# lionelblonde/sac-td3-cudagraphs-pytorch

Hardware: AMD Instinct MI355X
Metric: gradient-steps/sec (SAC, batch=256) at 1 GPU + 8-seed node; replay HBM GB/s (higher is better)
Workload: dtype f32; 1 GPU; SAC Hopper-v4 batch=256 2x256 MLP+LN, 100000 rows in a 1000000-row HBM ring, 1 critic update+Polyak per iteration, 2 actor+alpha updates every 3rd, hipGraph per 3 iterations; parallelism=1 independent seeds, one per GPU, no collective

## Files before the change

### sac-td3-cudagraphs-pytorch_amd/csrc/engine.hip

```cpp
#include <hip/hip_runtime.h>

#include <algorithm>
#include <cmath>
#include <cstdio>
#include <cstdlib>
#include <cstring>
#include <string>
#include <chrono>
#include <vector>

#include "../../include/sactd3.h"
#include "kernels.h"

static thread_local std::string g_create_error;

static inline int round_up(int x, int m) { return (x + m - 1) / m * m; }
static inline unsigned magic_div(unsigned d, unsigned long long n_max) {
  return (d > 1 && n_max * d < (1ull << 32)) ? (unsigned)(((1ull << 32) + d - 1) / d) : 0u;
}

static NetLayout make_layout(int K, int nh) {
  NetLayout L{};
  L.K = K; L.ld1 = round_up(K, 4); L.nh = nh;
  int off = 0;
// ... 52 lines not shown

  int o = 0, a = 0, B = 0, ldc = 0, ldo = 0, a4 = 0, nh = 0, ldu = 0, rec_f = 0, rec4 = 0, cx = 0, cn = 0;
  int nq_actor = 2;
  int nblk = 0, nblk4 = 0;
  AlphaArgs pending_alpha{}; bool alpha_pending = false;
  bool alpha_tick_owed = false;
  int maxn = 0;
  int num_cus = 256;
  int stage_rows = 0;
  NetLayout La{}, Lc{};

  DevCtl* ctl = nullptr;
  float *min_ac = nullptr, *max_ac = nullptr, *scale = nullptr, *bias = nullptr;
  float *Pa = nullptr, *Ta = nullptr, *Ga = nullptr, *Ma = nullptr, *Va = nullptr;
  float *Ta2 = nullptr, *Ta3 = nullptr;
  float *Pc = nullptr, *Tc = nullptr, *Gc = nullptr, *Mc = nullptr, *Vc = nullptr;
  float *la = nullptr, *gscale = nullptr;
  float* ring = nullptr; float* stage_dev = nullptr;
  float *X = nullptr, *Xn = nullptr, *Xp = nullptr, *rew = nullptr, *done = nullptr;
  int* idx = nullptr;
  float *logp_n = nullptr, *logp_pi = nullptr, *logp_al = nullptr, *act_scratch = nullptr;
  float* eps[SACTD3_NUM_SITES] = {};
  float *a_z1 = nullptr, *a_xh1 = nullptr, *a_h1 = nullptr, *a_rs1 = nullptr, *a_z2 = nullptr, *a_xh2 = nullptr, *a_h2 = nullptr, *a_rs2 = nullptr, *a_tg = nullptr;
  float *a_du = nullptr, *a_dz2 = nullptr, *a_dh1 = nullptr, *a_dz1 = nullptr;
  float *qa_ps = nullptr, *qa_S = nullptr;
  float *a_ps = nullptr, *c_ps = nullptr;
  float* a_z2n = nullptr;
  float* ah_z1[4] = {}; float* ah_z2[4] = {};
  struct BatchSlot { float *X, *Xn, *rew, *done, *logp_n, *eps_c; int* idx; } bs[4] = {};
  int cur_slot = 0;
  int chain_ready = -1;
  float *c_z1 = nullptr, *c_xh1 = nullptr, *c_h1 = nullptr, *c_rs1 = nullptr, *c_z2 = nullptr, *c_dz2 = nullptr, *c_dh1 = nullptr, *c_dz1 = nullptr;
  float *t_z1 = nullptr, *t_z2 = nullptr, *q = nullptr, *qt = nullptr, *y = nullptr, *q_pi = nullptr, *dA = nullptr;
  float* s_h1 = nullptr;
  float* Gp = nullptr; int gp_slabs = 0;
  float *part = nullptr, *part_s = nullptr, *part_sa = nullptr;
  float *p_x = nullptr, *p_z1 = nullptr, *p_z2 = nullptr, *p_act = nullptr;
  float *h_obs = nullptr, *h_act = nullptr;
  int* h_done = nullptr; int predict_calls = 0;
  float* h_stage[NSTAGE] = {}; int stage_next = 0, stage_used = 0;
  float* h_batch = nullptr;

  int64_t rb_len = 0, rb_cursor = 0, qnet_updates = 0;
  hipGraphExec_t graphs[G_COUNT] = {}; int graph_nodes[G_COUNT] = {};
  std::vector<hipGraphExec_t> predict_graphs;
  int tune_ks = 0, tune_nt = 0, tune_tn_kt = 0, tune_pad64 = 0, tune_tn64_min = 0, tune_rows4 = 0, tune_nn16 = 0, tune_xr = -1;
  int node_seq = 0, node_only = -1;
  const char* node_role = "";
  std::vector<NodeInfo>* node_log = nullptr;

  int fail(int code, const char* what, hipError_t he = hipSuccess) {
    err = what;
    if (he != hipSuccess) { err += ": "; err += hipGetErrorString(he); }
    return code;
  }
};

#define HIPCHK(call)                                                   \
  do {                                                                 \
    hipError_t _he = (call);                                           \
    if (_he != hipSuccess) return e->fail(SACTD3_EHIP, #call, _he);    \
  } while (0)
#define USE_DEVICE(e)                                                                        \
  do {                                                                                       \
    hipError_t _he = hipSetDevice((e)->cfg.device_id);                                       \
    if (_he != hipSuccess) return (e)->fail(SACTD3_EHIP, "hipSetDevice", _he);               \
    (void)hipGetLastError();    \
  } while (0)
#define CHAIN_BREAK(e) do { (e)->chain_ready = -1; } while (0)
#define RCCHK(call)                    \
  do {                                 \
    int _rc = (call);                  \
    if (_rc != 0) return _rc;          \
  } while (0)

template <class T>
static int dalloc(sactd3_engine* e, T** p, size_t count, bool zero = true) {
  void* v = nullptr;
  HIPCHK(hipMalloc(&v, std::max<size_t>(count, 4) * sizeof(T)));
  e->dev_allocs.push_back(v);
  if (zero) HIPCHK(hipMemset(v, 0, std::max<size_t>(count, 4) * sizeof(T)));
  *p = (T*)v;
  return 0;
}
template <class T>
static int halloc(sactd3_engine* e, T** p, size_t count) {
  void* v = nullptr;
  HIPCHK(hipHostMalloc(&v, std::max<size_t>(count, 4) * sizeof(T), hipHostMallocDefault));
  e->host_allocs.push_back(v);
  memset(v, 0, std::max<size_t>(count, 4) * sizeof(T));
  *p = (T*)v;
  return 0;
}

static inline bool node_on(sactd3_engine* e, const char* name, double flops, double bytes, dim3 grid, dim3 block) {
  if (e->node_only < 0 && !e->node_log) return true;
  const int k = e->node_seq++;
  if (e->node_log) {
    std::string n(name), detail;
    const size_t dot = n.find('.');
    if (dot != std::string::npos) { detail = "/" + n.substr(dot + 1); n.resize(dot); }
    e->node_log->push_back(NodeInfo{n + ":" + e->node_role + detail, flops, bytes,
                                    (long)grid.x * grid.y * grid.z * block.x * block.y * block.z});
  }
  return e->node_only < 0 || e->node_only == k;
}
#define LAUNCH_DYN(name, flops, bytes, kernel, grid, block, dyn_lds, ...)    \
  do {                                                                      \
    if (node_on(e, name, flops, bytes, grid, block)) {                      \
      hipLaunchKernelGGL(kernel, grid, block, dyn_lds, s, __VA_ARGS__);     \
      HIPCHK(hipGetLastError());                                            \
    }                                                                       \
  } while (0)
#define LAUNCH(name, flops, bytes, kernel, grid, block, ...) LAUNCH_DYN(name, flops, bytes, kernel, grid, block, 0, __VA_ARGS__)

static inline dim3 tile_grid(int tiles, int nets) { return dim3((unsigned)((tiles + 3) / 4), 1, (unsigned)nets); }

static unsigned gather_blocks(long chunks) {
  const long one = (chunks + 255) / 256;
  return (unsigned)(one <= 4096 ? one : (chunks + 256L * GATHER_CPT - 1) / (256L * GATHER_CPT));
}
static GatherArgs gather_args(sactd3_engine* e, const float* ring, int identity_len, int slot = 0, int ctr_add = 0) {
  GatherArgs g{};
  const sactd3_engine::BatchSlot& S = e->bs[slot];
  g.ring = (const float4*)ring; g.rec4 = e->rec4; g.cx = e->cx; g.cn = e->cn; g.ctl = e->ctl; g.idx = S.idx;
  g.X = (float4*)S.X; g.Xn = (float4*)S.Xn; g.rew = S.rew; g.done = S.done;
  g.B = e->B; g.len_override = identity_len; g.ctr_add = ctr_add;
  g.rec4_magic = magic_div((unsigned)e->rec4, (unsigned long long)e->B * e->rec4 + 1);
  const long chunks = (long)e->B * e->rec4;
  g.cpb = (int)((chunks + 256L * gather_blocks(chunks) - 1) / (256L * gather_blocks(chunks)));
  return g;
}
template <int PRO, bool F1, int C1>
static void launch_nt_ks(hipStream_t s, int ks, dim3 grid, const NtArgs& g) {
  if (ks == 4) hipLaunchKernelGGL((k_nt<PRO, F1, 4, C1>), grid, dim3(256), 0, s, g);
  else if (ks == 2) hipLaunchKernelGGL((k_nt<PRO, F1, 2, C1>), grid, dim3(256), 0, s, g);
  else hipLaunchKernelGGL((k_nt<PRO, F1, 1, C1>), grid, dim3(256), 0, s, g);
}
template <int PRO>
static void launch_nt_f1(hipStream_t s, int ks, int nt, dim3 grid, const NtArgs& g) {
  const int c1 = (g.K1 + 15) / 16;
  if (nt == 2) {
    if (c1 <= 1) hipLaunchKernelGGL((k_nt<PRO, true, 2, 1, 2>), grid, dim3(256), 0, s, g);
    else if (c1 == 2) hipLaunchKernelGGL((k_nt<PRO, true, 2, 2, 2>), grid, dim3(256), 0, s, g);
    else hipLaunchKernelGGL((k_nt<PRO, true, 2, 4, 2>), grid, dim3(256), 0, s, g);
    return;
  }
  if (c1 <= 1) launch_nt_ks<PRO, true, 1>(s, ks, grid, g);
  else if (c1 == 2) launch_nt_ks<PRO, true, 2>(s, ks, grid, g);
  else launch_nt_ks<PRO, true, 4>(s, ks, grid, g);
}
static void launch_nt_c4(hipStream_t s, int nt, dim3 grid, const NtArgs& g) {
  const int c1 = (g.K1 + 15) / 16;
  if (nt == 2) {
    if (c1 <= 1) hipLaunchKernelGGL((k_nt<1, true, 2, 1, 2, true>), grid, dim3(256), 0, s, g);
    else if (c1 == 2) hipLaunchKernelGGL((k_nt<1, true, 2, 2, 2, true>), grid, dim3(256), 0, s, g);
    else hipLaunchKernelGGL((k_nt<1, true, 2, 4, 2, true>), grid, dim3(256), 0, s, g);
  } else {
    if (c1 <= 1) hipLaunchKernelGGL((k_nt<1, true, 2, 1, 1, true>), grid, dim3(256), 0, s, g);
    else if (c1 == 2) hipLaunchKernelGGL((k_nt<1, true, 2, 2, 1, true>), grid, dim3(256), 0, s, g);
    else hipLaunchKernelGGL((k_nt<1, true, 2, 4, 1, true>), grid, dim3(256), 0, s, g);
  }
}
static int pick_xr(const sactd3_engine* e, int R, int C, double A, double W) {
  if (e->tune_xr >= 0) return (e->tune_xr == 0 || (R % e->tune_xr == 0 && C % (8 / e->tune_xr) == 0)) ? e->tune_xr : 0;
  int best = 0; double cost = 1e300;
  for (int xr = 1; xr <= 8; xr *= 2) {
    const int xc = 8 / xr;
    if (R % xr || C % xc) continue;
    const double c = xc * A + xr * W;
    if (c < cost) { cost = c; best = xr; }
  }
  return best;
}
static int launch_nt(sactd3_engine* e, hipStream_t s, const char* name, int pro, bool fuse1, const NtArgs& g, int nets, int force_ks = 0) {
  const int tiles_m = (g.M + 15) / 16, tiles_n = (g.N + 15) / 16;
  const double fl = 2.0 * nets * (double)g.M * g.N * (g.K + (fuse1 ? g.K1 : 0));
  double by = 4.0 * ((double)nets * g.N * (g.K + 3) + (double)nets * g.M * g.N);
  by += fuse1 ? 4.0 * ((double)nets * HID * (g.K1 + 1) + (double)(nets / g.npg) * g.M * g.K1) : 4.0 * (double)nets * g.M * g.K;
  for (int i = 0; i < nets / g.npg; ++i) by += 4.0 * g.npg * (double)g.M * HID * ((g.g[i].xh_out ? 1 : 0) + (g.g[i].h_out ? 1 : 0));
  if (g.gblocks) by += (g.gblocks / std::max(g.gb_each, 1)) * 8.0 * (double)g.ga[0].B * 4 * (g.ga[0].cx + g.ga[0].cn + 1);
  if (pro == 0) {
    const dim3 grid((unsigned)(tiles_m * tiles_n), 1, (unsigned)nets);
    if (!node_on(e, "k_nt_wide.layer1", fl, by, grid, dim3(256))) return 0;
    hipLaunchKernelGGL(k_nt_wide, grid, dim3(256), 0, s, g);
  } else {
    const int tiles = tiles_m * tiles_n * nets;
    int ks = tiles >= 2 * e->num_cus ? 2 : 4;
    if (e->tune_ks) ks = e->tune_ks;
    if (force_ks) ks = force_ks;
    const bool c4 = force_ks == 4 && fuse1 && pro == 1 && tiles >= 2 * e->num_cus && !(e->tune_rows4 & 32768);
    if (c4) ks = 2;
    const int rb = 64 / ks;
    int nt = (ks == 2 && ((g.M + rb - 1) / rb) * tiles_n * nets >= 2 * e->num_cus && tiles_n % 2 == 0) ? 2 : 1;
    if (e->tune_nt == 1 || (force_ks && !c4)) nt = 1;
    if (c4 && nt == 2 && ((g.M + rb - 1) / rb) * (tiles_n / 2) * nets > e->num_cus) nt = 1;
    NtArgs gg = g;
    gg.nt_blocks = ((g.M + rb - 1) / rb) * (tiles_n / nt);
    gg.xr = fuse1 ? 0 : pick_xr(e, (g.M + rb - 1) / rb, tiles_n / nt, 4.0 * g.M * g.K, 4.0 * g.N * g.K);
    int nzb = 0;
    for (int i = 0; i < gg.nz_n && i < 5; ++i) nzb += gg.nz[i].blocks;
    const int riders = gg.gblocks + gg.alpha_block + nzb;
    gg.flat = (nets > 1 && gg.alpha_block && riders <= 8 && !(e->tune_rows4 & 65536)) ? nets : 0;
    gg.flat_r = gg.flat ? (riders + 7) & ~7 : 0; gg.flat_n = riders;
    const dim3 grid = gg.flat ? dim3((unsigned)(gg.nt_blocks * nets + gg.flat_r)) : dim3((unsigned)(gg.nt_blocks + riders), 1, (unsigned)nets);
    char inst[64] = "k_nt";
    if (e->node_log) {
      const int c1 = (g.K1 + 15) / 16;
      snprintf(inst, sizeof(inst), c4 ? "k_nt<%d,%s,%d,%d,%d,true>.%s" : "k_nt<%d,%s,%d,%d,%d>.%s", pro, fuse1 ? "true" : "false", ks, fuse1 ? (c1 <= 1 ? 1 : (c1 == 2 ? 2 : 4)) : 0, nt, name);
    }
    if (!node_on(e, inst, fl, by, grid, dim3(256))) return 0;
    if (c4) launch_nt_c4(s, nt, grid, gg);
    else if (fuse1) { if (pro == 1) launch_nt_f1<1>(s, ks, nt, grid, gg); else launch_nt_f1<2>(s, ks, nt, grid, gg); }
    else if (nt == 2) {
      if (pro == 1) hipLaunchKernelGGL((k_nt<1, false, 2, 0, 2>), grid, dim3(256), 0, s, gg);
      else hipLaunchKernelGGL((k_nt<2, false, 2, 0, 2>), grid, dim3(256), 0, s, gg);
    } else { if (pro == 1) launch_nt_ks<1, false, 0>(s, ks, grid, gg); else launch_nt_ks<2, false, 0>(s, ks, grid, gg); }
  }
  HIPCHK(hipGetLastError());
  return 0;
}
static int launch_nn(sactd3_engine* e, hipStream_t s, const char* name, const NnArgs& g, int nets) {
  if (g.M >= BIG_BATCH && g.Kout == HID && g.k_off == 0 && !e->tune_nn16) {
    const double fl = 2.0 * nets * (double)g.M * HID * HID, by = 4.0 * nets * (2.0 * g.M * HID + (double)HID * HID);
    if (nets >= 2) {
      const dim3 grid((unsigned)(((g.M + 31) / 32) * (HID / 64) * nets));
      LAUNCH("k_nn64<2,2,2>.dh1", fl, by, (k_nn64<2, 2, 2>), grid, dim3(256), g);
    } else {
      const dim3 grid((unsigned)(((g.M + 31) / 32) * (HID / 32) * nets));
      LAUNCH("k_nn64<2,2,1>.dh1", fl, by, (k_nn64<2, 2, 1>), grid, dim3(256), g);
    }
    (void)name;
    return 0;
  }
  const dim3 grid((unsigned)(((g.M + 15) / 16) * ((g.Kout + 15) / 16)), 1, (unsigned)nets);
  NnArgs gg = g;
  gg.xr = pick_xr(e, (g.M + 15) / 16, (g.Kout + 15) / 16, 4.0 * g.M * HID, 4.0 * HID * g.Kout);
  LAUNCH(name, 2.0 * nets * (double)g.M * HID * g.Kout, 4.0 * nets * ((double)g.M * HID + (double)HID * g.Kout + (double)g.M * g.Kout),
         k_nn, grid, dim3(256), gg);
  return 0;
}
#ifndef TN64_CFG
#define TN64_CFG 2, 2, 2, 1, 64
#define TN64_N 64
#define TN64_K 32
#define TN64_M 64
#endif
#define TN64_KERNEL (k_tn64<TN64_CFG>)
static int launch_tn64(sactd3_engine* e, hipStream_t s, const char* name, const TnArgs& g, int nets, int tick_extra = 0) {
  Tn64Args a{};
  a.nprob = g.nprob; a.M = g.M; a.nets = nets; a.Gp = e->Gp; a.g_ns = nets > 1 ? g.g_ns : (long)e->La.size;
  AdamRedArgs r{};
  r.s_off = -1;
  int tiles = 0;
  double fl = 0.0, by = 0.0;
  for (int i = 0; i < g.nprob; ++i) {
    const TnProb& q = g.pr[i];
    Tn64Prob& t = a.pr[i];
    t.dY = q.dY; t.ldy = q.ldy; t.dy_ns = q.dy_ns; t.N = q.N; t.X = q.X; t.ldx = q.ldx; t.x_ns = q.x_ns; t.K = q.K;
    t.w_off = q.w_off; t.ldw = q.ldw; t.b_off = q.b_off;
    t.tiles_n = (q.N + TN64_N - 1) / TN64_N; t.tiles_k = (q.ldw + TN64_K - 1) / TN64_K; t.tile0 = tiles;
    tiles += t.tiles_n * t.tiles_k;
    for (int f = 0; f < q.nfin; ++f) { r.vec[r.nvec].off = q.fin_off[f]; r.vec[r.nvec].slot = q.fin_slot[f]; r.vec[r.nvec].nblk = q.fin_nblk[f]; ++r.nvec; }
    if (q.fin_s_off >= 0) { r.s_off = q.fin_s_off; r.s_nblk = q.fin_s_nblk; }
    fl += 2.0 * nets * (double)g.M * q.N * q.K;
    by += 4.0 * nets * (double)g.M * (q.N + q.K);
  }
  a.tiles_per_net = tiles;
  const int nch = (g.M + TN64_M - 1) / TN64_M;
  int S = (2 * e->num_cus + tiles * nets / 2) / (tiles * nets);
  S = std::max(1, std::min(S, std::min(e->gp_slabs, nch)));
  a.S = S;
  const long size = a.g_ns;
  {
    const dim3 grid((unsigned)(tiles * nets * S));
    char inst[96];
    snprintf(inst, sizeof(inst), "k_tn64<2,2,2,1,64>.dW(split-M x%d)", S);
    LAUNCH(inst, fl, by + 4.0 * S * nets * (double)size, TN64_KERNEL, grid, dim3(256), a);
  }
  r.Gp = e->Gp; r.S = S; r.nets = nets; r.g_ns = size; r.G = g.G;
  r.apply = g.apply; r.P = g.P; r.Mo = g.Mo; r.Vo = g.Vo; r.T = g.T; r.tau = g.tau; r.adam = g.adam; r.b1 = g.b1; r.b2 = g.b2; r.eps = g.eps;
  r.part = g.part; r.pstride = g.pstride; r.part_s = g.part_s;
  r.loss_part = g.loss_part; r.loss_n = g.loss_n; r.loss_stride = g.loss_stride; r.loss_off = g.loss_off; r.loss_scale = g.loss_scale;
  r.loss_dst = g.loss_dst; r.tick = g.tick; r.tick_extra = tick_extra;
  const dim3 grid((unsigned)((size / 4 + 255) / 256 + 4 * r.nvec + 1), (unsigned)nets);
  LAUNCH(g.apply ? (g.T ? "k_adam_red.sum+adam+polyak" : "k_adam_red.sum+adam") : "k_adam_red.sum", 0.0,
         nets * (double)size * (4.0 * S + 4.0 + (g.apply ? 24.0 : 0.0) + (g.apply && g.T ? 8.0 : 0.0)), k_adam_red, grid, dim3(256), r);
  (void)name;
  return 0;
}

static inline int tn_width(const TnProb& q) { return q.kw > 0 ? q.kw : q.ldw; }
static int launch_tn(sactd3_engine* e, hipStream_t s, const char* name, TnArgs& g, int nets, int tick_extra = 0) {
  if (g.M >= BIG_BATCH && e->Gp && !e->tune_tn_kt) {
    int tiles = 0;
    for (int i = 0; i < g.nprob; ++i) tiles += ((g.pr[i].N + TN64_N - 1) / TN64_N) * ((g.pr[i].ldw + TN64_K - 1) / TN64_K);
    if (tiles * nets >= e->tune_tn64_min) return launch_tn64(e, s, name, g, nets, tick_extra);
  }
  auto count = [&](int kt) {
    int tiles = 0;
    for (int i = 0; i < g.nprob; ++i) {
      g.pr[i].tile0 = tiles;
      tiles += ((g.pr[i].N + 15) / 16) * (((tn_width(g.pr[i]) + 15) / 16 + kt - 1) / kt);
    }
    return tiles;
  };
  int kt = (count(1) * nets > 2 * e->num_cus && g.M < BIG_BATCH) ? 2 : 1;
  if (e->tune_tn_kt) kt = e->tune_tn_kt;
  const int tiles = count(kt);
  for (int i = 0; i < g.nprob; ++i)
    g.pr[i].xr = g.pr[i].xr_force ? g.pr[i].xr_force
                                  : pick_xr(e, (g.pr[i].N + 15) / 16, ((tn_width(g.pr[i]) + 15) / 16 + kt - 1) / kt, 4.0 * g.M * g.pr[i].N, 4.0 * g.M * tn_width(g.pr[i]));
  double fl = 0.0, by = 0.0;
  for (int i = 0; i < g.nprob; ++i) {
    fl += 2.0 * nets * (double)g.M * g.pr[i].N * g.pr[i].K;
    by += 4.0 * nets * (double)g.M * ((g.pr[i].x_dup == 2 ? 0 : g.pr[i].N) + (g.pr[i].x_dup == 1 ? 0 : g.pr[i].K)) + (4.0 + (g.apply ? 24.0 : 0.0) + (g.apply && g.T ? 8.0 : 0.0)) * nets * (double)g.pr[i].N * (g.pr[i].K + 1);
  }
  bool fold = false;
  for (int i = 0; i < g.nprob; ++i) fold = fold || g.pr[i].fold;
  char inst[96];
  snprintf(inst, sizeof(inst), fold ? "k_tn<%d,true>.%s" : "k_tn<%d>.%s", kt, name);
  g.tiles = tiles;
  if (g.pk_blocks) by += 12.0 * (g.pk.n0 + g.pk.n1);
  {
    AdamRedArgs& r = g.fin;
    r = AdamRedArgs{};
    r.s_off = -1;
    for (int i = 0; i < g.nprob; ++i) {
      const TnProb& q = g.pr[i];
      for (int f = 0; f < q.nfin; ++f) { r.vec[r.nvec].off = q.fin_off[f]; r.vec[r.nvec].slot = q.fin_slot[f]; r.vec[r.nvec].nblk = q.fin_nblk[f]; ++r.nvec; }
      if (q.fin_s_off >= 0) { r.s_off = q.fin_s_off; r.s_nblk = q.fin_s_nblk; }
    }
    r.nets = nets; r.g_ns = g.g_ns; r.G = g.G;
    r.apply = g.apply; r.P = g.P; r.Mo = g.Mo; r.Vo = g.Vo; r.T = g.T; r.tau = g.tau; r.adam = g.adam; r.b1 = g.b1; r.b2 = g.b2; r.eps = g.eps;
    r.T2 = g.T2; r.T3 = g.T3;
    r.part = g.part; r.pstride = g.pstride; r.part_s = g.part_s;
    r.loss_part = g.loss_part; r.loss_n = g.loss_n; r.loss_stride = g.loss_stride; r.loss_off = g.loss_off; r.loss_scale = g.loss_scale;
    r.loss_dst = g.loss_dst; r.tick = g.tick; r.tick_extra = tick_extra;
    g.fin_blocks = 4 * r.nvec + 1;
  }
  const dim3 grid((unsigned)((tiles + g.pk_blocks + g.fin_blocks + (nets > 1 ? 7 : 0)) & (nets > 1 ? ~7 : ~0)), 1, (unsigned)nets);
  if (!node_on(e, inst, fl, by, grid, dim3(256))) return 0;
  if (fold) {
    if (kt == 2) hipLaunchKernelGGL((k_tn<2, true>), grid, dim3(256), 0, s, g);
    else hipLaunchKernelGGL((k_tn<1, true>), grid, dim3(256), 0, s, g);
  } else if (kt == 2) hipLaunchKernelGGL(k_tn<2>, grid, dim3(256), 0, s, g);
  else hipLaunchKernelGGL(k_tn<1>, grid, dim3(256), 0, s, g);
  HIPCHK(hipGetLastError());
  return 0;
}
static TnProb tn_prob(const float* dY, int ldy, long dy_ns, int N, const float* X, int ldx, long x_ns, int K,
                      int w_off, int ldw, int b_off) {
  TnProb q{};
  q.dY = dY; q.ldy = ldy; q.dy_ns = dy_ns; q.N = N; q.X = X; q.ldx = ldx; q.x_ns = x_ns; q.K = K;
  q.w_off = w_off; q.ldw = ldw; q.b_off = b_off; q.nfin = 0; q.fin_s_off = -1;
  return q;
// ... 1581 lines not shown
```

### sac-td3-cudagraphs-pytorch_amd/csrc/kernels.h

```cpp
#pragma once
#include <hip/hip_runtime.h>
#include <stdint.h>
#include <type_traits>
#include "philox.h"

#define HID 256
#define LN_EPS 1e-5f
#define NSLOT 5
#define AS 260
#define WS 68
#define YS 20

typedef float f32x4 __attribute__((ext_vector_type(4)));

#ifdef SACTD3_STAMPS
__device__ long long g_stamps[16];
__device__ long long g_phase[8];
#define PHASE_DECL long long ph_t = 0, ph_acc[6] = {0, 0, 0, 0, 0, 0}
#define PHASE_START do { __builtin_amdgcn_s_waitcnt(0xc07f); ph_t = clock64(); } while (0)
#define PHASE(i) do { const long long n_ = clock64(); ph_acc[i] += n_ - ph_t; ph_t = n_; } while (0)
#define PHASE_DRAIN(i) do { __builtin_amdgcn_s_waitcnt(0); const long long n_ = clock64(); ph_acc[i] += n_ - ph_t; ph_t = n_; } while (0)
#define PHASE_OUT do { if (threadIdx.x == 0 && blockIdx.x == gridDim.x - 1) for (int i_ = 0; i_ < 6; ++i_) g_phase[i_] = ph_acc[i_]; } while (0)
#define STAMP(i) do { if (threadIdx.x == 0 && blockIdx.x == gridDim.x - 1 && blockIdx.y == 0 && blockIdx.z == 0) { __builtin_amdgcn_s_waitcnt(0); g_stamps[i] = clock64(); } } while (0)
__device__ long long g_blk[4096 * 2];
// ... 238 lines not shown
  __shared__ int ids_s[GATHER_CPT * 256 + 2];
  const int inject = p.ctl->inject_idx, rb_len = p.ctl->rb_len, ctr = p.ctl->sample_ctr + p.ctr_add;
  const unsigned long long seed = p.ctl->seed;
  const int len = p.len_override >= 0 ? p.len_override : rb_len;
  const unsigned total = (unsigned)p.B * (unsigned)p.rec4;
  const unsigned c0 = block * (unsigned)p.cpb * 256u;
  if (c0 >= total) return;
  const unsigned c1 = min(c0 + (unsigned)p.cpb * 256u, total);
  const unsigned r0 = fast_div(c0, (unsigned)p.rec4, p.rec4_magic), r1 = fast_div(c1 - 1u, (unsigned)p.rec4, p.rec4_magic);
  for (unsigned i = threadIdx.x; i <= r1 - r0; i += 256u)
    ids_s[i] = inject ? p.idx[r0 + i] : (int)philox_index(seed, (unsigned)ctr, r0 + i, (unsigned)len);
  __syncthreads();
  int bb[GATHER_CPT], cc[GATHER_CPT], ids[GATHER_CPT]; float4 v[GATHER_CPT]; bool on[GATHER_CPT], first[GATHER_CPT];
#pragma unroll
  for (int u = 0; u < GATHER_CPT; ++u) {
    const unsigned g = c0 + (unsigned)u * 256u + threadIdx.x;
    on[u] = u < p.cpb && g < c1;
    const unsigned q = on[u] ? fast_div(g, (unsigned)p.rec4, p.rec4_magic) : r0;
    bb[u] = (int)q; cc[u] = on[u] ? (int)(g - q * (unsigned)p.rec4) : 0;
    ids[u] = ids_s[q - r0];
    first[u] = !inject && on[u] && cc[u] == 0;
    on[u] = on[u] && cc[u] <= p.cx + p.cn;
  }
#pragma unroll
  for (int u = 0; u < GATHER_CPT; ++u) v[u] = p.ring[(long)ids[u] * p.rec4 + (on[u] ? cc[u] : 0)];
#pragma unroll
  for (int u = 0; u < GATHER_CPT; ++u) {
    if (first[u]) p.idx[bb[u]] = ids[u];
    if (!on[u]) continue;
    const int b = bb[u], c = cc[u];
    if (c < p.cx) p.X[(long)b * p.cx + c] = v[u];
    else if (c < p.cx + p.cn) p.Xn[(long)b * p.cx + (c - p.cx)] = v[u];
    else { p.rew[b] = v[u].x; p.done[b] = v[u].y; }
  }
}
__global__ __launch_bounds__(256) void k_gather(GatherArgs p) { gather_body(p, blockIdx.x); }

__global__ void k_tick(int* a, int* b) {
  if (threadIdx.x == 0 && blockIdx.x == 0) { if (a) *a += 1; if (b) *b += 1; }
}
__global__ void k_set_int2(int* dst, int v0, int v1) {
  if (threadIdx.x == 0 && blockIdx.x == 0) { dst[0] = v0; dst[1] = v1; }
}

struct IngestArgs { const float4* src; float4* ring; int rec4, n, cursor, cap; int* len_cursor; int new_len, new_cursor; };
__global__ __launch_bounds__(256) void k_rb_ingest(IngestArgs p) {
  const int total = p.n * p.rec4;
  for (int g = blockIdx.x * 256 + threadIdx.x; g < total; g += gridDim.x * 256) {
    const int row = g / p.rec4, c = g - row * p.rec4;
    int dst = p.cursor + row;
    if (dst >= p.cap) dst -= p.cap;
    p.ring[(long)dst * p.rec4 + c] = p.src[g];
  }
  if (blockIdx.x == 0 && threadIdx.x == 0) { p.len_cursor[0] = p.new_len; p.len_cursor[1] = p.new_cursor; }
}

struct FillArgs { float4* ring; int rec4, cx, cn, o, a; long n; unsigned long long seed; const float* min_ac; const float* max_ac; };
__global__ __launch_bounds__(256) void k_rb_fill(FillArgs p) {
  const long g = (long)blockIdx.x * 256 + threadIdx.x;
  const long row = g / p.rec4; const int c = (int)(g % p.rec4);
  if (row >= p.n) return;
  const Philox4 r = philox4x32_10((uint32_t)row, (uint32_t)(row >> 32), SACTD3_STREAM_FILL, (uint32_t)c,
                                  (uint32_t)p.seed, (uint32_t)(p.seed >> 32));
  float nrm[4], uni[4];
  {
    const float u0 = philox_u01(r.v[0]), u1 = philox_u01(r.v[1]), u2 = philox_u01(r.v[2]), u3 = philox_u01(r.v[3]);
    const float r0 = sqrtf(-2.f * logf(u0)), r1 = sqrtf(-2.f * logf(u2));
    nrm[0] = r0 * cosf(6.283185307179586f * u1); nrm[1] = r0 * sinf(6.283185307179586f * u1);
    nrm[2] = r1 * cosf(6.283185307179586f * u3); nrm[3] = r1 * sinf(6.283185307179586f * u3);
    uni[0] = u0; uni[1] = u1; uni[2] = u2; uni[3] = u3;
  }
  float out[4] = {0.f, 0.f, 0.f, 0.f};
  if (c < p.cx) {
    for (int i = 0; i < 4; ++i) {
      const int e = 4 * c + i;
      if (e < p.o) out[i] = nrm[i];
      else if (e < p.o + p.a) { const int j = e - p.o; out[i] = p.min_ac[j] + (p.max_ac[j] - p.min_ac[j]) * uni[i]; }
    }
  } else if (c < p.cx + p.cn) {
    for (int i = 0; i < 4; ++i) if (4 * (c - p.cx) + i < p.o) out[i] = nrm[i];
  } else if (c == p.cx + p.cn) {
    out[0] = nrm[0];
    out[1] = uni[1] < 0.01f ? 1.f : 0.f;
  }
  p.ring[row * p.rec4 + c] = make_float4(out[0], out[1], out[2], out[3]);
}

__device__ __forceinline__ float f4c(const float4& v, int i) { return i == 0 ? v.x : (i == 1 ? v.y : (i == 2 ? v.z : v.w)); }
#define MFMA4(acc, a, b)                                                   \
  acc = __builtin_amdgcn_mfma_f32_16x16x4f32((a).x, (b).x, acc, 0, 0, 0);  \
  acc = __builtin_amdgcn_mfma_f32_16x16x4f32((a).y, (b).y, acc, 0, 0, 0);  \
  acc = __builtin_amdgcn_mfma_f32_16x16x4f32((a).z, (b).z, acc, 0, 0, 0);  \
  acc = __builtin_amdgcn_mfma_f32_16x16x4f32((a).w, (b).w, acc, 0, 0, 0);

struct AlphaArgs {
  const float* logp; int B; float targ_ent; int autotune;
  float* la;
  DevCtl* ctl; float lr, b1, b2, eps;
  int* tick;
};
__device__ __forceinline__ void alpha_body(const AlphaArgs& a) {
  __shared__ float red[8];
  const bool lead = threadIdx.x == 0;
  float la = 0.f, m = 0.f, v = 0.f; int tl = 0, tk = 0; double q0 = 0.0, q1 = 0.0;
  if (lead) {
    la = a.la[0];
    if (a.autotune) { m = a.la[1]; v = a.la[2]; tl = a.ctl->t_l; q0 = a.ctl->pw_l[0]; q1 = a.ctl->pw_l[1]; }
    if (a.tick) tk = *a.tick;
  }
  float s = 0.f;
  if (a.autotune && threadIdx.x < 256)
    for (int i = threadIdx.x; i < a.B; i += 256) s += -a.logp[i] - a.targ_ent;
  s = wave_sum(s);
  if ((threadIdx.x & 63) == 0) red[(threadIdx.x >> 6) & 7] = s;
  __syncthreads();
  if (lead) {
    if (a.autotune) {
      const float mean_term = ((red[0] + red[1]) + (red[2] + red[3])) / (float)a.B;
      const float g = expf(la) * mean_term;
      a.ctl->metrics[2] = g;
      const double p1 = q0 * (double)a.b1, p2 = q1 * (double)a.b2;
      a.ctl->t_l = tl + 1; a.ctl->pw_l[0] = p1; a.ctl->pw_l[1] = p2;
      const float sc0 = (float)((double)a.lr / (1.0 - p1)), sc1 = (float)sqrt(1.0 - p2);
      m = m + (g - m) * (1.0f - a.b1);
      v = v * a.b2 + g * g * (1.0f - a.b2);
      la -= sc0 * (m / (sqrtf(v) / sc1 + a.eps));
      a.la[0] = la; a.la[1] = m; a.la[2] = v;
    }
    a.ctl->metrics[3] = expf(la);
    if (a.tick) *a.tick = tk + 1;
  }
}
__global__ __launch_bounds__(256) void k_alpha_step(AlphaArgs a) { alpha_body(a); }

struct NtGrp {
  const float* in;
  const float* P;
  float* Y;
  float* xh_out; float* h_out; float* rstd_out;
  int ring; int ring_off; int sctr_add; const int* ring_idx;
};
struct NtArgs {
  NtGrp g[5]; int npg;
  int ld_in; long in_ns;
  int oW, ldw, oBias, oG, oBe; long p_ns;
  int ldy; long y_ns;
  int M, N, K;
  int K1, oW1, ldw1, oB1;
  long act_ns;
  int* tick0; int* tick1;
  float* adam_out; double* adam_pw; float lr, b1, b2;
  unsigned w1_magic;
  int nt_blocks; int gblocks; int gb_each;
  int flat, flat_r, flat_n;
  GatherArgs ga[3];
  int* tick0b; float* adam_out_b; double* adam_pw_b; float lr_b;
  int xr;
  int ln_pro;
  int alpha_block; AlphaArgs al;
  int nz_n; NoiseJob nz[5]; const DevCtl* nz_ctl;
};

__device__ __forceinline__ f32x4 splitk_reduce(float* red , f32x4 acc, int wave, int lane) {
  st4(red + (wave * 64 + lane) * 4, make_float4(acc[0], acc[1], acc[2], acc[3]));
  __syncthreads();
  f32x4 o = {0.f, 0.f, 0.f, 0.f};
  if (wave == 0) {
    const float4 a = ld4(red + lane * 4), b = ld4(red + (64 + lane) * 4), c = ld4(red + (128 + lane) * 4), d = ld4(red + (192 + lane) * 4);
    o[0] = (a.x + b.x) + (c.x + d.x); o[1] = (a.y + b.y) + (c.y + d.y);
    o[2] = (a.z + b.z) + (c.z + d.z); o[3] = (a.w + b.w) + (c.w + d.w);
  }
  return o;
}

__device__ __forceinline__ void riding_body(const NtArgs& p, int x) {
  if (x < p.alpha_block) { alpha_body(p.al); return; }
  x -= p.alpha_block;
  if (x < p.nz[0].blocks) { noise_body(p.nz[0], p.nz_ctl, x); return; }
  x -= p.nz[0].blocks;
  if (p.nz_n > 1 && x < p.nz[1].blocks) { noise_body(p.nz[1], p.nz_ctl, x); return; }
  x -= p.nz[1].blocks;
  if (p.nz_n > 2 && x < p.nz[2].blocks) { noise_body(p.nz[2], p.nz_ctl, x); return; }
  x -= p.nz[2].blocks;
  if (p.nz_n > 3 && x < p.nz[3].blocks) { noise_body(p.nz[3], p.nz_ctl, x); return; }
  x -= p.nz[3].blocks;
  if (p.nz_n > 4) noise_body(p.nz[4], p.nz_ctl, x);
}
__device__ __forceinline__ void riding_gather(const NtArgs& p, int x) {
  if (x < p.gb_each) gather_body(p.ga[0], x);
  else if (x < 2 * p.gb_each) gather_body(p.ga[1], x - p.gb_each);
  else gather_body(p.ga[2], x - 2 * p.gb_each);
}

template <int PRO, bool FUSE1, int KS, int C1, int NT = 1, bool C4 = false>
__global__ __launch_bounds__(256) void k_nt(NtArgs p) {
  static_assert(!C4 || (KS == 2 && PRO == 1), "C4: the KS = 2 LayerNorm form only");
  constexpr int RB = 64 / KS, CW = 16 / KS, NP = C4 ? 16 : 4 * KS, SS = 2 * NP + 4;
  constexpr int W1S = 16 * (C1 > 0 ? C1 : 1) + 4;
  __shared__ __attribute__((aligned(16))) float W2s[NT * 16 * AS];
  __shared__ __attribute__((aligned(16))) float W1s[FUSE1 ? HID * W1S : 4];
  __shared__ __attribute__((aligned(16))) float vec[3 * HID];
  __shared__ __attribute__((aligned(16))) float stat[RB * SS];
  constexpr int RED = KS > 1 ? (C4 ? 2 : 1) * NT * 4 * 64 * 4 : 4;
  static_assert(!FUSE1 || RED <= HID * W1S, "red fits W1's slab");
  __shared__ __attribute__((aligned(16))) float red_own[FUSE1 ? 4 : RED];
  float* red = FUSE1 ? W1s : red_own;
  BLK_MARK_K(1, 0);
  int bx = blockIdx.x, net = blockIdx.z;
  bool rider_net0 = blockIdx.z == 0;
  if (p.flat) {
    rider_net0 = true;
    if (bx < p.flat_r) { if (bx >= p.flat_n) return; bx += p.nt_blocks; net = 0; }
    else { bx -= p.flat_r; net = small_div(bx, p.nt_blocks); bx -= net * p.nt_blocks; }
  }
  if ((p.gblocks || p.alpha_block || p.nz_n) && bx >= p.nt_blocks) {
    const int x = bx - p.nt_blocks;
    if (x < p.gblocks) { if (rider_net0) riding_gather(p, x); }
    else if (!rider_net0) { }
    else riding_body(p, x - p.gblocks);
    BLK_MARK_K(1, 1);
    return;
  }
  const int t = threadIdx.x, lane = t & 63, wave = t >> 6;
  const int r = lane & 15, kq = lane >> 4;
  const int mt = wave / KS, ks = wave % KS;
  if (bx == 0 && net == 0) {
    if (t == 0 && (p.tick0 || p.tick1)) tick_all(p.tick0, p.tick1, p.adam_pw, p.adam_out, p.lr, p.b1, p.b2);
    if (t == 64 && p.tick0b) tick_all(p.tick0b, nullptr, p.adam_pw_b, p.adam_out_b, p.lr_b, p.b1, p.b2);
  }
  const int grp = net / p.npg, ni = net - grp * p.npg;
  const NtGrp G = p.g[grp];
  const float* Pn = G.P + ni * p.p_ns;
  const int tiles_n = (p.N + 16 * NT - 1) / (16 * NT);
  int tmb, tn;
  xcd_tile(bx, (p.M + RB - 1) / RB, tiles_n, FUSE1 ? 0 : p.xr, tmb, tn);
  const int m0 = tmb * RB + 16 * mt, n0 = tn * 16 * NT;
  const int mrow = min(m0 + r, p.M - 1);
  const int kb = (ks * CW) * 16 + 4 * kq;
  float bias[NT];
#pragma unroll
  for (int nt = 0; nt < NT; ++nt) bias[nt] = p.oBias >= 0 ? Pn[p.oBias + min(n0 + 16 * nt + r, p.N - 1)] : 0.f;
  STAMP(0); BLK_PH_K(1, 0);
  float4 w2r[4 * NT], w1r[C1 > 0 ? 4 * C1 : 1], vr = f4(0.f), xv[C1 > 0 ? C1 : 1], av[CW];
  const int w1n = FUSE1 ? (HID * p.ldw1) >> 2 : 0;
  if (FUSE1) {
#pragma unroll
    for (int u = 0; u < 4 * C1; ++u) {
      const int f = min(t + 256 * u, w1n - 1);
      w1r[u] = ld4(Pn + p.oW1 + 4 * (long)f);
    }
    const float* xrow = G.in + ni * p.in_ns + (long)mrow * p.ld_in;
    if (G.ring) {
      const int inject = p.ga[0].ctl->inject_idx, rb_len = p.ga[0].ctl->rb_len, sctr = p.ga[0].ctl->sample_ctr + G.sctr_add;
      const unsigned long long seed = p.ga[0].ctl->seed;
      int id = (int)philox_index(seed, (unsigned)sctr, (unsigned)mrow, (unsigned)max(rb_len, 1));
      if (inject) id = G.ring_idx[mrow];
      xrow = reinterpret_cast<const float*>(p.ga[0].ring) + (long)id * (4 * p.ga[0].rec4) + G.ring_off;
    }
#pragma unroll
    for (int c1 = 0; c1 < C1; ++c1) {
      const int k = 16 * c1 + 4 * kq;
      xv[c1] = ld4_cols(xrow, k, p.K1, (p.K1 + 3) & ~3);
    }
  } else {
#pragma unroll
    for (int c = 0; c < CW; ++c) av[c] = ld4(G.in + ni * p.in_ns + (long)mrow * p.ld_in + kb + 16 * c);
  }
  if (t < 192) {
    const int which = t >> 6, c4 = t & 63;
    const int off = which == 0 ? p.oB1 : (which == 1 ? p.oG : p.oBe);
    if ((which == 0 && FUSE1) || (which != 0 && PRO == 1)) vr = ld4(Pn + off + 4 * c4);
  }
#pragma unroll
  for (int u = 0; u < 4 * NT; ++u) {
    const int i = t + 256 * u, row = i >> 6, c4 = i & 63, n = min(n0 + row, p.N - 1);
    w2r[u] = ld4(Pn + p.oW + (long)n * p.ldw + 4 * c4);
  }
  __builtin_amdgcn_sched_barrier(0);
  if (FUSE1) {
#pragma unroll
    for (int u = 0; u < 4 * C1; ++u) {
      const int f = t + 256 * u;
      if (f < w1n) { const int e = 4 * f, row = (int)fast_div((unsigned)e, (unsigned)p.ldw1, p.w1_magic), col = e - row * p.ldw1; st4(W1s + row * W1S + col, w1r[u]); }
    }
  }
  if (t < 192) st4(vec + 4 * t, vr);
  __syncthreads();
  STAMP(1); BLK_PH_K(1, 1);
  if (FUSE1) {
    constexpr int GT = CW < 4 ? CW : 4;
#pragma unroll
    for (int c0 = 0; c0 < CW; c0 += GT) {
      float4 wf[GT][C1 > 0 ? C1 : 1], b1[GT];
      f32x4 z[GT];
#pragma unroll
      for (int j = 0; j < GT; ++j) {
        const int tile = ks * CW + c0 + j;
#pragma unroll
        for (int c1 = 0; c1 < C1; ++c1) {
          const int k = 16 * c1 + 4 * kq;
          wf[j][c1] = k < p.ldw1 ? ld4(W1s + (tile * 16 + r) * W1S + k) : f4(0.f);
        }
        b1[j] = ld4(vec + tile * 16 + 4 * kq);
        z[j] = f32x4{0.f, 0.f, 0.f, 0.f};
      }
#pragma unroll
      for (int c1 = 0; c1 < C1; ++c1)
#pragma unroll
        for (int q = 0; q < 4; ++q)
#pragma unroll
          for (int j = 0; j < GT; ++j) z[j] = __builtin_amdgcn_mfma_f32_16x16x4f32(f4c(wf[j][c1], q), f4c(xv[c1], q), z[j], 0, 0, 0);
#pragma unroll
      for (int j = 0; j < GT; ++j) av[c0 + j] = make_float4(z[j][0] + b1[j].x, z[j][1] + b1[j].y, z[j][2] + b1[j].z, z[j][3] + b1[j].w);
    }
  }
#pragma unroll
  for (int u = 0; u < 4 * NT; ++u) { const int i = t + 256 * u; st4(W2s + (i >> 6) * AS + 4 * (i & 63), w2r[u]); }
  float4 xh[CW];
  float rstd = 1.f;
  if (PRO == 1) {
    constexpr int CG = C4 ? 4 : CW;
    constexpr float nl = 4.0f * CG;
    float* srow = stat + (16 * mt + r) * SS;
#pragma unroll
    for (int h = 0; h < CW / CG; ++h) {
      float ml = 0.f;
#pragma unroll
      for (int c = 0; c < CG; ++c) ml += sum4(av[CG * h + c]);
      ml *= (1.0f / nl);
      float m2 = 0.f;
#pragma unroll
      for (int c = 0; c < CG; ++c) { const float4 d = av[CG * h + c] - f4(ml); m2 += dot4(d, d); }
      const int slot = (C4 ? 2 * ks + h : ks) * 4 + kq;
      srow[2 * slot] = ml;
      srow[2 * slot + 1] = m2;
    }
    __syncthreads();
    float4 sp[NP / 2];
#pragma unroll
    for (int i = 0; i < NP / 2; ++i) sp[i] = ld4(srow + 4 * i);
    float mean = 0.f;
#pragma unroll
    for (int i = 0; i < NP / 2; ++i) mean += sp[i].x + sp[i].z;
    mean *= (1.0f / NP);
    float M2 = 0.f;
#pragma unroll
    for (int i = 0; i < NP / 2; ++i) {
      const float d0 = sp[i].x - mean, d1 = sp[i].z - mean;
      M2 += (sp[i].y + sp[i].w) + nl * (d0 * d0 + d1 * d1);
    }
    rstd = 1.0f / sqrtf(M2 * (1.0f / HID) + LN_EPS);
#pragma unroll
    for (int c = 0; c < CW; ++c) {
      const float4 gv = ld4(vec + HID + kb + 16 * c), bv = ld4(vec + 2 * HID + kb + 16 * c);
      xh[c] = (av[c] - f4(mean)) * rstd;
      av[c] = relu4(xh[c] * gv + bv);
    }
  } else {
    __syncthreads();
    if (PRO == 2) {
#pragma unroll
      for (int c = 0; c < CW; ++c) { xh[c] = av[c]; av[c] = relu4(av[c]); }
    }
  }
  STAMP(2); BLK_PH_K(1, 2);
  if (PRO != 0 && m0 + r < p.M) {
    const long ro = ni * p.act_ns + (long)(m0 + r) * HID + kb;
    const int gsz = 16 / tiles_n, g0 = tn * gsz;
#pragma unroll
    for (int c = 0; c < CW; ++c) {
      const int gc = ks * CW + c;
      if (gc >= g0 && gc < g0 + gsz) {
        if (G.xh_out) st4(G.xh_out + ro + 16 * c, xh[c]);
        if (G.h_out) st4(G.h_out + ro + 16 * c, av[c]);
      }
    }
    if (G.rstd_out && tn == 0 && ks == 0 && kq == 0) G.rstd_out[(long)ni * p.M + m0 + r] = rstd;
  }
  constexpr int NH = C4 ? 2 : 1;
  f32x4 acc[NT], ph[NT][NH];
  {
    constexpr int GC = CW < 4 ? CW : 4;
#pragma unroll
    for (int h = 0; h < NH; ++h) {
      f32x4 a0[NT], a1[NT];
#pragma unroll
      for (int nt = 0; nt < NT; ++nt) { a0[nt] = f32x4{0.f, 0.f, 0.f, 0.f}; a1[nt] = f32x4{0.f, 0.f, 0.f, 0.f}; }
#pragma unroll
      for (int c0 = h * (CW / NH); c0 < (h + 1) * (CW / NH); c0 += GC) {
        float4 wv[NT][GC];
#pragma unroll
        for (int nt = 0; nt < NT; ++nt)
#pragma unroll
          for (int j = 0; j < GC; ++j) wv[nt][j] = ld4(W2s + (16 * nt + r) * AS + kb + 16 * (c0 + j));
#pragma unroll
        for (int j = 0; j < GC; j += 2)
#pragma unroll
          for (int q = 0; q < 4; ++q)
#pragma unroll
            for (int nt = 0; nt < NT; ++nt) {
              a0[nt] = __builtin_amdgcn_mfma_f32_16x16x4f32(f4c(av[c0 + j], q), f4c(wv[nt][j], q), a0[nt], 0, 0, 0);
              if (j + 1 < GC) a1[nt] = __builtin_amdgcn_mfma_f32_16x16x4f32(f4c(av[c0 + j + 1], q), f4c(wv[nt][j + 1], q), a1[nt], 0, 0, 0);
            }
      }
#pragma unroll
      for (int nt = 0; nt < NT; ++nt) { ph[nt][h][0] = a0[nt][0] + a1[nt][0]; ph[nt][h][1] = a0[nt][1] + a1[nt][1]; ph[nt][h][2] = a0[nt][2] + a1[nt][2]; ph[nt][h][3] = a0[nt][3] + a1[nt][3]; }
    }
#pragma unroll
    for (int nt = 0; nt < NT; ++nt) acc[nt] = ph[nt][0];
  }
  STAMP(3); BLK_PH_K(1, 3);
  if (KS > 1) {
#pragma unroll
    for (int nt = 0; nt < NT; ++nt)
#pragma unroll
      for (int h = 0; h < NH; ++h)
        st4(red + (((nt * 4 + wave) * NH + h) * 64 + lane) * 4, make_float4(ph[nt][h][0], ph[nt][h][1], ph[nt][h][2], ph[nt][h][3]));
    __syncthreads();
    if (ks == 0) {
#pragma unroll
      for (int nt = 0; nt < NT; ++nt)
#pragma unroll
        for (int j = 0; j < KS; ++j)
#pragma unroll
          for (int h = 0; h < NH; ++h) {
            if (j == 0 && h == 0) continue;
            const float4 o = ld4(red + (((nt * 4 + wave + j) * NH + h) * 64 + lane) * 4);
            acc[nt][0] += o.x; acc[nt][1] += o.y; acc[nt][2] += o.z; acc[nt][3] += o.w;
          }
    }
  }
  STAMP(4); BLK_PH_K(1, 4);
  if (ks == 0) {
    float* y = G.Y + ni * p.y_ns;
#pragma unroll
    for (int nt = 0; nt < NT; ++nt) {
      const int col = n0 + 16 * nt + (lane & 15);
      if (col >= p.N) continue;
#pragma unroll
      for (int i = 0; i < 4; ++i) {
        const int row = m0 + 4 * (lane >> 4) + i;
        if (row < p.M) y[(long)row * p.ldy + col] = acc[nt][i] + bias[nt];
      }
    }
  }
  STAMP(5); BLK_PH_K(1, 5);
  BLK_MARK_K(1, 1);
}

__global__ __launch_bounds__(256) void k_nt_wide(NtArgs p) {
  __shared__ __attribute__((aligned(16))) float red[4 * 64 * 4];
  const int t = threadIdx.x, lane = t & 63, wave = t >> 6, net = blockIdx.z;
  const int r = lane & 15, kq = lane >> 4;
  if (blockIdx.x == 0 && t == 0 && net == 0) {
    if (p.tick0 || p.tick1) tick_all(p.tick0, p.tick1, p.adam_pw, p.adam_out, p.lr, p.b1, p.b2);
  }
  if (blockIdx.x == 0 && t == 64 && net == 0 && p.tick0b) tick_all(p.tick0b, nullptr, p.adam_pw_b, p.adam_out_b, p.lr_b, p.b1, p.b2);
  const int grp = net / p.npg, ni = net - grp * p.npg;
  const NtGrp G = p.g[grp];
  const float* Pn = G.P + ni * p.p_ns;
  const int tiles_n = (p.N + 15) >> 4;
  const int tm = blockIdx.x / tiles_n, tn = blockIdx.x % tiles_n;
  const int m0 = tm * 16, n0 = tn * 16;
  const float* Arow = G.in + ni * p.in_ns + (long)min(m0 + r, p.M - 1) * p.ld_in;
  const float* Wrow = Pn + p.oW + (long)min(n0 + r, p.N - 1) * p.ldw;
  const int chunks = (p.K + 15) >> 4, Kr = (p.K + 3) & ~3;
  float bias = p.oBias >= 0 ? Pn[p.oBias + min(n0 + r, p.N - 1)] : 0.f;
  f32x4 acc = {0.f, 0.f, 0.f, 0.f};
  for (int cb = 0; cb < chunks; cb += 32) {
    float4 a[8], w[8];
#pragma unroll
    for (int u = 0; u < 8; ++u) {
      const int c = cb + wave + 4 * u, k = 16 * c + 4 * kq;
      a[u] = ld4_cols(Arow, k, p.K, Kr);
      w[u] = ld4_cols(Wrow, k, p.K, Kr);
    }
    __builtin_amdgcn_sched_barrier(0);
#pragma unroll
    for (int u = 0; u < 8; ++u) { MFMA4(acc, a[u], w[u]); }
  }
  PIN(bias);
  acc = splitk_reduce(red, acc, wave, lane);
  const int col = n0 + (lane & 15);
  if (wave == 0 && col < p.N) {
    float* y = G.Y + ni * p.y_ns;
#pragma unroll
    for (int i = 0; i < 4; ++i) {
      const int row = m0 + 4 * (lane >> 4) + i;
      if (row < p.M) y[(long)row * p.ldy + col] = acc[i] + bias;
    }
  }
}

#define KC64 64
#define LS64 (KC64 + 4)
template <int WM, int WN, int TT>
__global__ __launch_bounds__(64 * WM * WN) void k_nt64(NtArgs p) {
  constexpr int TM = 16 * WM, TN = 16 * TT * WN, NTH = 64 * WM * WN;
  constexpr int RA = 16 * TM / NTH, RW = 16 * TN / NTH, SR = NTH / 16;
  static_assert(RA >= 1 && RW >= 1 && 16 * TM % NTH == 0 && 16 * TN % NTH == 0, "staging map");
  __shared__ __attribute__((aligned(16))) float As[2][TM * LS64];
  __shared__ __attribute__((aligned(16))) float Ws[2][TN * LS64];
  const int t = threadIdx.x, lane = t & 63, wave = t >> 6, wm = wave % WM, wn = wave / WM;
  const int r = lane & 15, kq = lane >> 4;
  const int tile_blocks = (p.gblocks || p.alpha_block) ? p.nt_blocks : (int)gridDim.x;
  if ((int)blockIdx.x >= tile_blocks) {
    const int x = (int)blockIdx.x - tile_blocks;
    if (NTH == 256 && x < p.gblocks) riding_gather(p, x);
    else if (x >= p.gblocks && p.alpha_block) alpha_body(p.al);
    return;
  }
  if (blockIdx.x == 0 && t == 0) {
    if (p.tick0 || p.tick1) tick_all(p.tick0, p.tick1, p.adam_pw, p.adam_out, p.lr, p.b1, p.b2);
  }
  if (blockIdx.x == 0 && t == 64 && p.tick0b) tick_all(p.tick0b, nullptr, p.adam_pw_b, p.adam_out_b, p.lr_b, p.b1, p.b2);
  const int tiles_n = (p.N + TN - 1) / TN, tiles = tiles_n * ((p.M + TM - 1) / TM);
  int L = blockIdx.x;
  { const int per = tile_blocks >> 3; if (L < per * 8) L = (L & 7) * per + (L >> 3); }
  const int net = L / tiles, idx = L - net * tiles;
  const int grp = net / p.npg, ni = net - grp * p.npg;
  const NtGrp G = p.g[grp];
  const float* Pn = G.P + ni * p.p_ns;
  const float* A = G.in + ni * p.in_ns;
  const int bm = idx / tiles_n, bn = idx - bm * tiles_n;
  const int m0 = bm * TM, n0 = bn * TN;
  const int sr0 = t >> 4, sc = (t & 15) * 4;
  const float* ap[RA]; const float* wp[RW];
#pragma unroll
  for (int u = 0; u < RA; ++u) ap[u] = A + (long)min(m0 + sr0 + SR * u, p.M - 1) * p.ld_in;
  if (G.ring) {
    const int inject = p.ga[0].ctl->inject_idx, rb_len = p.ga[0].ctl->rb_len, sctr = p.ga[0].ctl->sample_ctr + G.sctr_add;
    const unsigned long long seed = p.ga[0].ctl->seed;
    int inj_id[RA];
#pragma unroll
    for (int u = 0; u < RA; ++u) inj_id[u] = G.ring_idx[min(m0 + sr0 + SR * u, p.M - 1)];
    __builtin_amdgcn_sched_barrier(0);
#pragma unroll
    for (int u = 0; u < RA; ++u) {
      const int m = min(m0 + sr0 + SR * u, p.M - 1);
      const int drawn = (int)philox_index(seed, (unsigned)sctr, (unsigned)m, (unsigned)max(rb_len, 1));
      const int id = inject ? min(max(inj_id[u], 0), max(rb_len, 1) - 1) : drawn;
      ap[u] = reinterpret_cast<const float*>(p.ga[0].ring) + (long)id * (4 * p.ga[0].rec4) + G.ring_off;
    }
  }
#pragma unroll
  for (int u = 0; u < RW; ++u) wp[u] = Pn + p.oW + (long)min(n0 + sr0 + SR * u, p.N - 1) * p.ldw;
  const int Kr = (p.K + 3) & ~3;
  f32x4 acc[TT];
#pragma unroll
  for (int tt = 0; tt < TT; ++tt) acc[tt] = f32x4{0.f, 0.f, 0.f, 0.f};
  const int nc = (p.K + KC64 - 1) / KC64;
  float bias[TT];
#pragma unroll
  for (int tt = 0; tt < TT; ++tt) bias[tt] = p.oBias >= 0 ? Pn[p.oBias + min(n0 + 16 * TT * wn + 16 * tt + r, p.N - 1)] : 0.f;
  float4 ra[RA], rw[RW];
  auto fetch = [&](int c) {
    const int k = c * KC64 + sc;
#pragma unroll
    for (int u = 0; u < RA; ++u) ra[u] = ld4_raw(ap[u], k, Kr);
#pragma unroll
    for (int u = 0; u < RW; ++u) rw[u] = ld4_raw(wp[u], k, Kr);
  };
  auto park = [&](int buf, int c) {
    const int k = c * KC64 + sc;
#pragma unroll
    for (int u = 0; u < RA; ++u) st4(As[buf] + (sr0 + SR * u) * LS64 + sc, mask4_cols(ra[u], k, p.K));
#pragma unroll
    for (int u = 0; u < RW; ++u) st4(Ws[buf] + (sr0 + SR * u) * LS64 + sc, mask4_cols(rw[u], k, p.K));
  };
  STAMP(0);
  fetch(0);
  park(0, 0);
  __syncthreads();
  for (int c = 0; c < nc; ++c) {
    const int buf = c & 1;
    if (c + 1 < nc) fetch(c + 1);
    __builtin_amdgcn_sched_barrier(0);
    const float* ab = As[buf] + (16 * wm + r) * LS64 + 4 * kq;
    const float* wb = Ws[buf] + (16 * TT * wn + r) * LS64 + 4 * kq;
#pragma unroll
// ... 2153 lines not shown
```

Before: 18880 gradient-steps/s.

## Add three-N-tile C4 variant of fused layer kernel with rebalanced gather riders

Adds an NT=3 instantiation of the C4 fused-first-layer kernel, chosen when two N-tiles per block would oversubscribe the CUs and K1<=16. It handles uneven tile splits for the xh/h output stores, resizes the gather rider blocks, and places the flat rider blocks after the GEMM blocks. In the C4 path the split-K reduction now writes only non-zero ks partials to LDS and keeps the ks==0 partial in registers, which halves the reduction buffer. The aim is to fit the grid in a single wave of CUs instead of falling back to NT=1. The cost is higher register pressure per block and more complex indexing.

```diff
diff --git a/sac-td3-cudagraphs-pytorch_amd/csrc/engine.hip b/sac-td3-cudagraphs-pytorch_amd/csrc/engine.hip
--- a/sac-td3-cudagraphs-pytorch_amd/csrc/engine.hip
+++ b/sac-td3-cudagraphs-pytorch_amd/csrc/engine.hip
@@ -228,7 +228,8 @@
 }
 static void launch_nt_c4(hipStream_t s, int nt, dim3 grid, const NtArgs& g) {
   const int c1 = (g.K1 + 15) / 16;
-  if (nt == 2) {
+  if (nt == 3) hipLaunchKernelGGL((k_nt<1, true, 2, 1, 3, true>), grid, dim3(256), 0, s, g);
+  else if (nt == 2) {
     if (c1 <= 1) hipLaunchKernelGGL((k_nt<1, true, 2, 1, 2, true>), grid, dim3(256), 0, s, g);
     else if (c1 == 2) hipLaunchKernelGGL((k_nt<1, true, 2, 2, 2, true>), grid, dim3(256), 0, s, g);
     else hipLaunchKernelGGL((k_nt<1, true, 2, 4, 2, true>), grid, dim3(256), 0, s, g);
@@ -270,14 +271,24 @@
     const int rb = 64 / ks;
     int nt = (ks == 2 && ((g.M + rb - 1) / rb) * tiles_n * nets >= 2 * e->num_cus && tiles_n % 2 == 0) ? 2 : 1;
     if (e->tune_nt == 1 || (force_ks && !c4)) nt = 1;
-    if (c4 && nt == 2 && ((g.M + rb - 1) / rb) * (tiles_n / 2) * nets > e->num_cus) nt = 1;
+    const int rows_b = (g.M + rb - 1) / rb;
+    if (c4 && nt == 2 && rows_b * (tiles_n / 2) * nets > e->num_cus)
+      nt = (g.K1 <= 16 && rows_b * ((tiles_n + 2) / 3) * nets <= e->num_cus && !(e->tune_rows4 & 524288)) ? 3 : 1;
     NtArgs gg = g;
-    gg.nt_blocks = ((g.M + rb - 1) / rb) * (tiles_n / nt);
+    gg.nt_blocks = rows_b * ((tiles_n + nt - 1) / nt);
     gg.xr = fuse1 ? 0 : pick_xr(e, (g.M + rb - 1) / rb, tiles_n / nt, 4.0 * g.M * g.K, 4.0 * g.N * g.K);
+    if (nt == 3 && gg.gblocks) {
+      const long chunks = (long)gg.ga[0].B * gg.ga[0].rec4;
+      const int ng = gg.gblocks / gg.gb_each;
+      gg.gb_each = (int)((chunks + 256L * GATHER_CPT - 1) / (256L * GATHER_CPT));
+      for (int i = 0; i < ng; ++i) gg.ga[i].cpb = (int)((chunks + 256L * gg.gb_each - 1) / (256L * gg.gb_each));
+      gg.gblocks = ng * gg.gb_each;
+    }
     int nzb = 0;
     for (int i = 0; i < gg.nz_n && i < 5; ++i) nzb += gg.nz[i].blocks;
     const int riders = gg.gblocks + gg.alpha_block + nzb;
     gg.flat = (nets > 1 && gg.alpha_block && riders <= 8 && !(e->tune_rows4 & 65536)) ? nets : 0;
+    if (nt == 3 && riders) { gg.flat = nets; gg.flat_at = gg.nt_blocks * nets; }
     gg.flat_r = gg.flat ? (riders + 7) & ~7 : 0; gg.flat_n = riders;
     const dim3 grid = gg.flat ? dim3((unsigned)(gg.nt_blocks * nets + gg.flat_r)) : dim3((unsigned)(gg.nt_blocks + riders), 1, (unsigned)nets);
     char inst[64] = "k_nt";
diff --git a/sac-td3-cudagraphs-pytorch_amd/csrc/kernels.h b/sac-td3-cudagraphs-pytorch_amd/csrc/kernels.h
--- a/sac-td3-cudagraphs-pytorch_amd/csrc/kernels.h
+++ b/sac-td3-cudagraphs-pytorch_amd/csrc/kernels.h
@@ -414,7 +414,7 @@
   float* adam_out; double* adam_pw; float lr, b1, b2;
   unsigned w1_magic;
   int nt_blocks; int gblocks; int gb_each;
-  int flat, flat_r, flat_n;
+  int flat, flat_r, flat_n, flat_at;
   GatherArgs ga[3];
   int* tick0b; float* adam_out_b; double* adam_pw_b; float lr_b;
   int xr;
@@ -463,7 +463,7 @@
   __shared__ __attribute__((aligned(16))) float W1s[FUSE1 ? HID * W1S : 4];
   __shared__ __attribute__((aligned(16))) float vec[3 * HID];
   __shared__ __attribute__((aligned(16))) float stat[RB * SS];
-  constexpr int RED = KS > 1 ? (C4 ? 2 : 1) * NT * 4 * 64 * 4 : 4;
+  constexpr int RED = KS > 1 ? NT * 4 * 64 * 4 : 4;
   static_assert(!FUSE1 || RED <= HID * W1S, "red fits W1's slab");
   __shared__ __attribute__((aligned(16))) float red_own[FUSE1 ? 4 : RED];
   float* red = FUSE1 ? W1s : red_own;
@@ -472,8 +472,9 @@
   bool rider_net0 = blockIdx.z == 0;
   if (p.flat) {
     rider_net0 = true;
-    if (bx < p.flat_r) { if (bx >= p.flat_n) return; bx += p.nt_blocks; net = 0; }
-    else { bx -= p.flat_r; net = small_div(bx, p.nt_blocks); bx -= net * p.nt_blocks; }
+    const int x = bx - p.flat_at;
+    if (x >= 0 && x < p.flat_r) { if (x >= p.flat_n) return; bx = x + p.nt_blocks; net = 0; }
+    else { if (x >= 0) bx -= p.flat_r; net = small_div(bx, p.nt_blocks); bx -= net * p.nt_blocks; }
   }
   if ((p.gblocks || p.alpha_block || p.nz_n) && bx >= p.nt_blocks) {
     const int x = bx - p.nt_blocks;
@@ -628,11 +629,11 @@
   STAMP(2); BLK_PH_K(1, 2);
   if (PRO != 0 && m0 + r < p.M) {
     const long ro = ni * p.act_ns + (long)(m0 + r) * HID + kb;
-    const int gsz = 16 / tiles_n, g0 = tn * gsz;
+    const int g0 = NT == 3 ? small_div(16 * tn, tiles_n) : tn * (16 / tiles_n), g1 = NT == 3 ? small_div(16 * tn + 16, tiles_n) : g0 + 16 / tiles_n;
 #pragma unroll
     for (int c = 0; c < CW; ++c) {
       const int gc = ks * CW + c;
-      if (gc >= g0 && gc < g0 + gsz) {
+      if (gc >= g0 && gc < g1) {
         if (G.xh_out) st4(G.xh_out + ro + 16 * c, xh[c]);
         if (G.h_out) st4(G.h_out + ro + 16 * c, av[c]);
       }
@@ -676,8 +677,11 @@
 #pragma unroll
     for (int nt = 0; nt < NT; ++nt)
 #pragma unroll
-      for (int h = 0; h < NH; ++h)
-        st4(red + (((nt * 4 + wave) * NH + h) * 64 + lane) * 4, make_float4(ph[nt][h][0], ph[nt][h][1], ph[nt][h][2], ph[nt][h][3]));
+      for (int h = 0; h < NH; ++h) {
+        const float4 v = make_float4(ph[nt][h][0], ph[nt][h][1], ph[nt][h][2], ph[nt][h][3]);
+        if (!C4) st4(red + (((nt * 4 + wave) * NH + h) * 64 + lane) * 4, v);
+        else if (ks != 0) st4(red + (((nt * 2 + mt) * NH + h) * 64 + lane) * 4, v);
+      }
     __syncthreads();
     if (ks == 0) {
 #pragma unroll
@@ -687,7 +691,9 @@
 #pragma unroll
           for (int h = 0; h < NH; ++h) {
             if (j == 0 && h == 0) continue;
-            const float4 o = ld4(red + (((nt * 4 + wave + j) * NH + h) * 64 + lane) * 4);
+            const float4 o = !C4 ? ld4(red + (((nt * 4 + wave + j) * NH + h) * 64 + lane) * 4)
+                           : j == 0 ? make_float4(ph[nt][h][0], ph[nt][h][1], ph[nt][h][2], ph[nt][h][3])
+                           : ld4(red + (((nt * 2 + mt) * NH + h) * 64 + lane) * 4);
             acc[nt][0] += o.x; acc[nt][1] += o.y; acc[nt][2] += o.z; acc[nt][3] += o.w;
           }
     }
```

New measurement: 19110 gradient-steps/s (median of 6 runs). +1.3%, better.
